# mazpie/genrl

Measured on AMD Instinct MI355X. Metric: world-model+imag update steps/sec (B32xL32x64x64x3), higher is better.
Workload: dtype f32 (storage, accumulation, every non-GEMM kernel and the fp32-MFMA GEMMs; the forward / dgrad / weight-gradient products of the imagination rollout, of the Dense+LN+SiLU chains from 192 rows up and of the encoder / decoder convolutions take fp32 operands pre-split into two fp16 planes of the scaled

## Files before the change

### genrl_amd/csrc/gemm_planes_tn.hip

```cpp
#include "common.h"
#include "genrl_hip.h"
#include <type_traits>

typedef _Float16 tn_f16x8 __attribute__((ext_vector_type(8)));
typedef _Float16 tn_f16x4 __attribute__((ext_vector_type(4)));

namespace {

struct TnArgs {
  const u16* a; long a_ld, a_plane;
  const u16* b; long b_ld, b_plane;
  const u16* fac;
  long fac_stride;
  const float* cref;
  float* out; long ldo; long split_stride;
  const float* bias_unused;
  int NI, NJ, M, stages_per_split, accumulate, tiles_i, tiles_j;
  const unsigned* rowoff; int cW, cC, ck;
};

__device__ __forceinline__ void tn_glds16(const void* g, unsigned lds_byte_addr) {
  __builtin_amdgcn_global_load_lds((const __attribute__((address_space(1))) void*)g,
                                   (__attribute__((address_space(3))) void*)(uintptr_t)lds_byte_addr, 16, 0, 0);
}
// ... 158 lines not shown
    const int s = u / (NPL * TN), p = (u / TN) % NPL, j = u % TN;
    fr[set][s][TM + j][p] = fr[set][s][TM + j][p] * fc[set][s];
  };
  auto mfma_one = [&](int set, int m) __attribute__((always_inline)) {
    constexpr int PA[3] = {1, 0, 0}, PB[3] = {0, 0, 1}, CL[3] = {0, 1, 0};
    const int s = m / (3 * TM * TN), t = (m / (TM * TN)) % 3, i = (m / TN) % TM, j = m % TN;
    acc[CL[t]][i][j] = __builtin_amdgcn_mfma_f32_32x32x16_f16(fr[set][s][TM + j][PB[t]], fr[set][s][i][PA[t]], acc[CL[t]][i][j], 0, 0, 0);
  };

  int left = nk, fleft = nk2;
  bool first = true;
  auto next_stage = [&]() __attribute__((always_inline)) {
    if (!first) {
      if (left > 0 && !(CONVB && isB)) gbase += stage_bytes;
      if (fleft > 0) fbase += BK * 2;
    }
    first = false;
    --left; --fleft;
  };
  auto issue_one = [&](int buf, int i) __attribute__((always_inline)) {
    if (i < NPD) {
      if constexpr (CONVB) {
        if (isB) { tn_glds16(gbase + (size_t)(ro[buf][i] + tapoff), piece0 + buf * STAGE + i * 1024); return; }
      }
      tn_glds16(gbase + (size_t)voff[i], piece0 + buf * STAGE + i * 1024);
    } else tn_glds4(fbase, fslot + buf * STAGE);
  };
  if constexpr (CONVB) {
    load_ro(std::integral_constant<int, 0>{});
    load_ro(std::integral_constant<int, 1>{});
    tn_wait_vm<0>();
    __builtin_amdgcn_sched_barrier(0);
  }
#pragma unroll
  for (int st = 0; st < NS; ++st) {
    next_stage();
#pragma unroll
    for (int i = 0; i < NP; ++i) issue_one(st, i);
  }
  next_stage();
  if constexpr (CONVB) {
    load_ro(std::integral_constant<int, 0>{});
    tn_wait_vm<0>();
  } else {
    tn_wait_vm<(NS - 1) * NP>();
  }
  __builtin_amdgcn_s_barrier();
  [&]<int... R>(std::integer_sequence<int, R...>) __attribute__((always_inline)) {
    (read_one(std::integral_constant<int, 0>{}, std::integral_constant<int, R>{}, std::integral_constant<int, 0>{}), ...);
  }(std::make_integer_sequence<int, TN_NR>{});
  asm volatile("s_waitcnt lgkmcnt(0)" ::: "memory");
  __builtin_amdgcn_sched_barrier(0);

  int it = 0;
  auto side_ops = [&](auto SET, auto Mc) __attribute__((always_inline)) {
    constexpr int set = decltype(SET)::value, m = decltype(Mc)::value, buf = set, buf1 = 1 - set;
    constexpr int lo = (m - TN_KB) * TN_PER;
    auto one = [&](auto Oc) __attribute__((always_inline)) {
      constexpr int o = decltype(Oc)::value;
      if constexpr (o < TN_NMEM) {
        if constexpr (tn_is_dma(o)) issue_one(buf, o / 3);
        else read_one(std::integral_constant<int, 1 - set>{}, std::integral_constant<int, (o < 3 * NP ? o - o / 3 : o - NP)>{},
                      std::integral_constant<int, buf1>{});
      }
    };
    one(std::integral_constant<int, lo>{});
    one(std::integral_constant<int, lo + 1>{});
    auto unit = [&](auto Uc) __attribute__((always_inline)) {
      constexpr int u = decltype(Uc)::value, rdy = tn_ready_of(u);
      if constexpr (rdy < TN_NM) {
        if constexpr (m == rdy) {
          constexpr int s_ = u / (NPL * TN), p_ = (u / TN) % NPL, j_ = u % TN;
          tn_wait_lgkm<tn_reads_through(m) - (tn_rlast_of(u) + 1)>(fr[1 - set][s_][TM + j_][p_], fc[1 - set][s_]);
          scale_one(1 - set, u);
        }
      } else {
        if constexpr (m == (rdy - TN_NM < TN_KB ? TN_KB : rdy - TN_NM)) scale_one(set, u);
      }
    };
    [&]<int... U>(std::integer_sequence<int, U...>) __attribute__((always_inline)) { (unit(std::integral_constant<int, U>{}), ...); }
    (std::make_integer_sequence<int, TN_NSC>{});
  };
  auto mfmas = [&](auto self, auto SET, auto Mc) __attribute__((always_inline)) -> void {
    constexpr int set = decltype(SET)::value, m = decltype(Mc)::value;
    if constexpr (m < TN_NM) {
      mfma_one(set, m);
      side_ops(SET, Mc);
      __builtin_amdgcn_sched_barrier(0);
      self(self, SET, std::integral_constant<int, m + 1>{});
    }
  };
  auto iteration = [&](auto SET) __attribute__((always_inline)) {
    constexpr int set = decltype(SET)::value;
    asm volatile("s_waitcnt lgkmcnt(0)" ::: "memory");
    __builtin_amdgcn_sched_barrier(0);
    mfma_one(set, 0);
    mfma_one(set, 1);
    __builtin_amdgcn_sched_barrier(0);
    tn_wait_vm<0>();
    __builtin_amdgcn_s_barrier();
    __builtin_amdgcn_sched_barrier(0);
    load_ro(std::integral_constant<int, 1 - set>{});
    __builtin_amdgcn_sched_barrier(0);
    mfmas(mfmas, SET, std::integral_constant<int, TN_KB>{});
    if constexpr (CONVB) { tn_wait_vm<NP>(); __builtin_amdgcn_sched_barrier(0); }
    next_stage();
    ++it;
  };
  [&]<int... U>(std::integer_sequence<int, U...>) __attribute__((always_inline)) {
    ([&](auto Uc) __attribute__((always_inline)) {
      constexpr int u = decltype(Uc)::value;
      if constexpr (tn_ready_of(u) < TN_NM) scale_one(0, u);
    }(std::integral_constant<int, U>{}), ...);
  }(std::make_integer_sequence<int, TN_NSC>{});
  while (it < nk2) {
    iteration(std::integral_constant<int, 0>{});
    iteration(std::integral_constant<int, 1>{});
  }
  tn_wait_vm<0>();

  const int l32 = lane & 31, h32 = lane >> 5;
  const float cr = g.cref[split];
  float* out = g.out + (long)split * g.split_stride;
  const bool vec = ((g.ldo & 3) == 0) && ((reinterpret_cast<uintptr_t>(out) & 15) == 0);
#pragma unroll
  for (int i = 0; i < TM; ++i) {
    const int row = i0 + (wm * TM + i) * 32 + l32;
    if (row >= g.NI) continue;
#pragma unroll
    for (int j = 0; j < TN; ++j)
#pragma unroll
      for (int gq = 0; gq < 4; ++gq) {
        const int col = j0 + (wn * TN + j) * 32 + 8 * gq + 4 * h32;
        if (col >= g.NJ) continue;
        float o[4];
#pragma unroll
        for (int v = 0; v < 4; ++v) o[v] = (acc[0][i][j][4 * gq + v] * (1.f / 2048.f) + acc[1][i][j][4 * gq + v]) * cr;
        float* c = out + (long)row * g.ldo + col;
        if (vec && col + 3 < g.NJ) {
          if (g.accumulate) {
            const float4 cv = *reinterpret_cast<const float4*>(c);
            o[0] += cv.x; o[1] += cv.y; o[2] += cv.z; o[3] += cv.w;
          }
          *reinterpret_cast<float4*>(c) = make_float4(o[0], o[1], o[2], o[3]);
        } else {
#pragma unroll
          for (int v = 0; v < 4; ++v)
            if (col + v < g.NJ) c[v] = o[v] + (g.accumulate ? c[v] : 0.f);
        }
      }
  }
}

__global__ __launch_bounds__(256) void tn_factors_kernel(const float* __restrict__ ia, const float* __restrict__ ib, int M,
                                                         int rows_per_split, long fac_stride, u16* __restrict__ fac,
                                                         float* __restrict__ cref) {
  __shared__ int red[4];
  const int r0 = blockIdx.x * rows_per_split, r1 = min(M, r0 + rows_per_split);
  auto efield = [](float v) { return (int)((__builtin_bit_cast(unsigned, v) >> 23) & 255u); };
  int emax = 0;
  for (int r = r0 + 4 * threadIdx.x; r < r1; r += 1024) {
    const float4 a = *reinterpret_cast<const float4*>(ia + r), b = *reinterpret_cast<const float4*>(ib + r);
    emax = max(max(max(efield(a.x) + efield(b.x), efield(a.y) + efield(b.y)), max(efield(a.z) + efield(b.z), efield(a.w) + efield(b.w))), emax);
  }
#pragma unroll
  for (int o = 32; o > 0; o >>= 1) emax = max(emax, __shfl_xor(emax, o, 64));
  if ((threadIdx.x & 63) == 0) red[threadIdx.x >> 6] = emax;
  __syncthreads();
  emax = max(max(red[0], red[1]), max(red[2], red[3]));
  if (threadIdx.x == 0) {
    const int e = min(max(emax - 254, -149), 127);
    cref[blockIdx.x] = ldexpf(1.0f, e);
  }
  auto f16_pow2 = [](int d) -> unsigned { return d >= -14 ? (unsigned)(d + 15) << 10 : (d >= -24 ? 1u << (d + 24) : 0u); };
  u16* f = fac + (long)blockIdx.x * fac_stride;
  for (int r = 4 * threadIdx.x; r < fac_stride; r += 1024) {
    unsigned lo = 0, hi = 0;
    if (r0 + r < r1) {
      const float4 a = *reinterpret_cast<const float4*>(ia + r0 + r), b = *reinterpret_cast<const float4*>(ib + r0 + r);
      lo = f16_pow2(efield(a.x) + efield(b.x) - emax) | (f16_pow2(efield(a.y) + efield(b.y) - emax) << 16);
      hi = f16_pow2(efield(a.z) + efield(b.z) - emax) | (f16_pow2(efield(a.w) + efield(b.w) - emax) << 16);
    }
    *reinterpret_cast<uint2*>(f + r) = make_uint2(lo, hi);
  }
}

__global__ __launch_bounds__(256) void tn_reduce_kernel(const float* __restrict__ part, long split_stride, int splits,
                                                        float* __restrict__ C, long ldc, int NI, int NJ, int accumulate) {
  const long n4 = (long)NI * (NJ / 4);
  for (long idx = (long)blockIdx.x * 256 + threadIdx.x; idx < n4; idx += (long)gridDim.x * 256) {
    const int row = (int)(idx / (NJ / 4)), c4 = (int)(idx % (NJ / 4));
    const float* p = part + (long)row * NJ + 4 * c4;
    float4 s = *reinterpret_cast<const float4*>(p);
    for (int k = 1; k < splits; ++k) {
      const float4 v = *reinterpret_cast<const float4*>(p + k * split_stride);
      s.x += v.x; s.y += v.y; s.z += v.z; s.w += v.w;
    }
    float* c = C + (long)row * ldc + 4 * c4;
    if (accumulate) { s.x += c[0]; s.y += c[1]; s.z += c[2]; s.w += c[3]; }
    c[0] = s.x; c[1] = s.y; c[2] = s.z; c[3] = s.w;
  }
}

int tn_splits(int NI, int NJ, int M) {
  const int tiles = cdiv(NI, 128) * cdiv(NJ, 128), stages = M / 64;
  int smax = stages / 8 > 0 ? stages / 8 : 1;
  if (smax > 64) smax = 64;
  int best = 1; long bc = -1;
  for (int s = 1; s <= smax; ++s) {
    const long cost = (long)cdiv((long)tiles * s, 256) * (cdiv(stages, s) + 8);
    if (bc < 0 || cost < bc) { bc = cost; best = s; }
  }
  return best;
}
struct TnPlan { int nsplit, sps; long fac_stride, fac_bytes; };
TnPlan tn_plan(int NI, int NJ, int M) {
  TnPlan p;
  const int splits = tn_splits(NI, NJ, M), stages = M / 64;
  p.sps = cdiv(stages, splits);
  p.nsplit = cdiv(stages, p.sps);
  p.fac_stride = (long)(((p.sps + 1) & ~1) * 64 + 128);
  p.fac_bytes = (p.nsplit * p.fac_stride * 2 + 255) / 256 * 256;
  return p;
}

}

extern unsigned g_planes_route;
extern int g_planes_route_splits;

extern "C" {

long genrl_gemm_h2_tn_ws_bytes(int NI, int NJ, int M) {
  if (NI <= 0 || NJ <= 0 || M <= 0) return 0;
  const TnPlan p = tn_plan(NI, NJ, M);
  long b = p.fac_bytes + 256;
  if (p.nsplit > 1) b += (long)p.nsplit * NI * ((NJ + 3) / 4 * 4) * 4;
  return b;
}

static int tn_impl(const uint16_t* a, long a_ld, long a_plane, const float* a_inv, const uint16_t* b, long b_ld, long b_plane,
                   const float* b_inv, float* C, long ldc, int NI, int NJ, int M, int accumulate, void* ws, long ws_bytes,
                   const unsigned* rowoff, int cW, int cC, int ck, void* stream) {
  GENRL_ENTER();
  if (NI <= 0 || NJ <= 0 || M <= 0 || (M & 63) || (a_ld & 63) || a_ld < NI || !a_inv || !b_inv || !ws) return GENRL_EINVAL;
  if (!rowoff && ((b_ld & 63) || b_ld < NJ)) return GENRL_EINVAL;
  if (rowoff && ((cC & 7) || (b_ld & 7) || b_ld < cC || (NJ & 7) || NJ != ck * ck * cC)) return GENRL_EINVAL;
  if (ws_bytes < genrl_gemm_h2_tn_ws_bytes(NI, NJ, M) || (reinterpret_cast<uintptr_t>(ws) & 255)) return GENRL_EINVAL;
  if ((reinterpret_cast<uintptr_t>(a_inv) | reinterpret_cast<uintptr_t>(b_inv)) & 15) return GENRL_EINVAL;
  hipStream_t s = (hipStream_t)stream;
  const TnPlan pl = tn_plan(NI, NJ, M);
  const int nsplit = pl.nsplit, sps = pl.sps;
  if (nsplit > 1 && ((NJ & 3) || (ldc & 3))) return GENRL_EINVAL;
  g_planes_route = rowoff ? GENRL_ROUTE_TN_CONV : GENRL_ROUTE_TN;
  g_planes_route_splits = nsplit;
  char* w = reinterpret_cast<char*>(ws);
  u16* fac = reinterpret_cast<u16*>(w);
  float* cref = reinterpret_cast<float*>(w + pl.fac_bytes);
  float* part = cref + 64;
  tn_factors_kernel<<<nsplit, 256, 0, s>>>(a_inv, b_inv, M, sps * 64, pl.fac_stride, fac, cref);
  GENRL_CHECK_LAUNCH();
  const int ti = cdiv(NI, 128), tj = cdiv(NJ, 128);
  const int NJp = (NJ + 3) / 4 * 4;
  TnArgs g{a, a_ld, a_plane, b, b_ld, b_plane, fac, pl.fac_stride, cref, nullptr, 0, 0, nullptr, NI, NJ, M, sps, 0, ti, tj,
           rowoff, cW, cC, ck};
  if (nsplit == 1) {
    g.out = C; g.ldo = ldc; g.split_stride = 0; g.accumulate = accumulate;
  } else {
    g.out = part; g.ldo = NJp; g.split_stride = (long)NI * NJp; g.accumulate = 0;
  }
  genrl_log_launch(rowoff ? "h2tn/conv" : "h2tn", NI, NJ, M,
                   4.0 * ((double)M * NI + (rowoff ? 4.0 * (double)M * cC : (double)M * NJ) + (double)NI * NJ));
  if (rowoff) gemm_planes_tn_kernel<true><<<ti * tj * nsplit, 256, 0, s>>>(g);
  else gemm_planes_tn_kernel<false><<<ti * tj * nsplit, 256, 0, s>>>(g);
  GENRL_CHECK_LAUNCH();
  if (nsplit > 1) {
    const long n4 = (long)NI * (NJ / 4);
    int nb = cdiv(n4, 256); if (nb > 2048) nb = 2048;
    tn_reduce_kernel<<<nb, 256, 0, s>>>(part, g.split_stride, nsplit, C, ldc, NI, NJ, accumulate);
    GENRL_CHECK_LAUNCH();
  }
  return GENRL_OK;
}

int genrl_gemm_h2_tn(const uint16_t* a, long a_ld, long a_plane, const float* a_inv, const uint16_t* b, long b_ld, long b_plane,
                     const float* b_inv, float* C, long ldc, int NI, int NJ, int M, int accumulate, void* ws, long ws_bytes,
                     void* stream) {
  g_planes_route = 0; g_planes_route_splits = 0;
  return tn_impl(a, a_ld, a_plane, a_inv, b, b_ld, b_plane, b_inv, C, ldc, NI, NJ, M, accumulate, ws, ws_bytes, nullptr, 0, 0, 0, stream);
}

int genrl_gemm_h2_tn_conv(const uint16_t* a, long a_ld, long a_plane, const float* a_inv, const uint16_t* img, long ld_img,
                          long plane_img, const float* img_inv, const unsigned* rowoff, int W, int Cc, int k, float* C, long ldc,
                          int NI, int M, int accumulate, void* ws, long ws_bytes, void* stream) {
  g_planes_route = 0; g_planes_route_splits = 0;
  if (!rowoff || k <= 0) return GENRL_EINVAL;
  return tn_impl(a, a_ld, a_plane, a_inv, img, ld_img, plane_img, img_inv, C, ldc, NI, k * k * Cc, M, accumulate, ws, ws_bytes, rowoff,
                 W, Cc, k, stream);
}

}
```

### genrl_amd/planes.py

```python
import ctypes
import os
import weakref
import torch
from ._lib import lib, check, GenrlHipError

ENABLED = os.environ.get('GENRL_PLANES', '1') != '0'
_amp_saved = None
gemm_profile = None


from .streams import raw_current_stream as _stream
from .streams import timed_start, timed_end


def r64(k):
    return (k + 63) // 64 * 64


class Planes:
    __slots__ = ('t', 'inv', 'rows', 'cols', 'ld', 'plane', 'uniform')

    def __init__(self, rows, cols, dev, zero=True):
        self.rows, self.cols, self.ld = rows, cols, r64(cols)
        self.uniform = False
# ... 71 lines not shown
        return
    arr = (_Desc * len(stale))()
    for d, ((_, transpose, c0, c1), ent) in zip(arr, stale):
        W, P = ent[3](), ent[1]
        d.src, d.ldx, d.R, d.Cn = W.data_ptr() + 4 * c0 * W.stride(1), W.stride(0), W.shape[0], c1 - c0
        d.out, d.ld_out, d.plane, d.inv, d.transpose = P.ptr(0), P.ld, P.plane, P.inv_ptr(0), int(transpose)
    check(lib().genrl_split_h2_batch(ctypes.cast(arr, ctypes.c_void_p), len(stale), stream), 'split_h2_batch')
    for _, ent in stale:
        ent[0], ent[2] = _epoch, ent[3]().data_ptr()


def _refresh_stale(stream):
    _split_entries([(key, ent) for key, ent in _wcache.items() if ent[0] != _epoch and ent[4] == stream and ent[3]() is not None], stream)


def refresh(params):
    ids = {id(q) for q in params}
    _split_entries([(key, ent) for key, ent in _wcache.items() if key[0] in ids and ent[3]() is not None], _stream())


def weight(W, transpose=False, c0=0, c1=None):
    c1 = W.shape[1] if c1 is None else c1
    if not isinstance(W, torch.nn.Parameter):
        return split(W.detach()[:, c0:c1], transpose)
    key = (id(W), transpose, c0, c1)
    ent = _wcache.get(key)
    st = _stream()
    if ent is None or ent[2] != W.data_ptr() or ent[3]() is not W:
        rows, cols = (c1 - c0, W.shape[0]) if transpose else (W.shape[0], c1 - c0)
        assert W.dim() == 2 and W.stride(1) == 1
        if ent is None:
            weakref.finalize(W, _wcache.pop, key, None)
        ent = _wcache[key] = [-1, Planes(rows, cols, W.device), W.data_ptr(), weakref.ref(W), st]
    ent[4] = st
    if ent[0] != _epoch:
        _refresh_stale(st)
    return ent[1]


def gemm(A, B, C, ldc, bias, M, N, accumulate=False, a_row0=0, A1=None, B1=None, a1_row0=0, c_off=0, b_row0=0, b1_row0=0):
    assert A.ld == B.ld and a_row0 + M <= A.rows and b_row0 + N <= B.rows, (A.ld, B.ld, A.rows, B.rows, M, N)
    e0 = timed_start(gemm_profile)
    k1 = 0
    a1 = b1 = (None, 0, 0, None)
    if A1 is not None:
        assert A1.ld == B1.ld and a1_row0 + M <= A1.rows and b1_row0 + N <= B1.rows
        k1 = A1.ld
        a1, b1 = (A1.ptr(a1_row0), A1.ld, A1.plane, A1.inv_ptr(a1_row0)), (B1.ptr(b1_row0), B1.ld, B1.plane, B1.inv_ptr(b1_row0))
    check(lib().genrl_gemm_h2(A.ptr(a_row0), A.ld, A.plane, A.inv_ptr(a_row0), B.ptr(b_row0), B.ld, B.plane, B.inv_ptr(b_row0),
                              A.ld, *a1, *b1, k1, C.data_ptr() + 4 * c_off, ldc, bias.data_ptr() if bias is not None else None,
                              M, N, int(accumulate), _stream()), 'gemm_h2')
    timed_end(gemm_profile, e0, M, N, A.cols + (A1.cols if A1 is not None else 0), 'kk/h2/pipe4')


LN_FUSED = os.environ.get('GENRL_GEMM_LN', '1') != '0'
_ln_ws = {}


def _ln_workspace(dev):
    d = torch.device(dev).index
    d = torch.cuda.current_device() if d is None else d
    ws = _ln_ws.get(d)
    if ws is None:
        if torch.cuda.is_current_stream_capturing():
            return None
        L = lib()
        ws = _ln_ws[d] = (torch.zeros(L.genrl_gemm_h2_ln_sync_words(), dtype=torch.int32, device=f'cuda:{d}'),
                          torch.zeros(L.genrl_gemm_h2_ln_part_floats(1024, 1024) + 4, device=f'cuda:{d}'))
    return ws


def ln_fused_here(dev=None):
    if not (LN_FUSED and ENABLED):
        return False
    from . import streams
    return not streams.on_side_stream() and _ln_workspace(dev if dev is not None else torch.cuda.current_device()) is not None


def gemm_ln_ok(M, N, dev=None):
    return LN_FUSED and ENABLED and lib().genrl_gemm_h2_ln_ok(M, N) == 1 and ln_fused_here(dev)


def gemm_ln(A, B, C, bias, M, N, gamma, beta, eps, out_p, out_row0, y=None, mean=None, rstd=None, act=True, a_row0=0, A1=None, B1=None,
            a1_row0=0, c_off=0, y_off=0, m_off=0):
    assert A.ld == B.ld and a_row0 + M <= A.rows and N <= B.rows and out_p.cols == N and out_row0 + M <= out_p.rows
    k1 = 0
    a1 = b1 = (None, 0, 0, None)
    if A1 is not None:
        assert A1.ld == B1.ld and a1_row0 + M <= A1.rows and N <= B1.rows
        k1 = A1.ld
        a1, b1 = (A1.ptr(a1_row0), A1.ld, A1.plane, A1.inv_ptr(a1_row0)), (B1.ptr(0), B1.ld, B1.plane, B1.inv_ptr(0))
    cptr = C.data_ptr() + 4 * c_off
    yptr = (y.data_ptr() + 4 * y_off) if y is not None else 0
    if (cptr | yptr | gamma.data_ptr() | beta.data_ptr() | (bias.data_ptr() if bias is not None else 0)) & 15:
        gemm(A, B, C, N, bias, M, N, a_row0=a_row0, A1=A1, B1=B1, a1_row0=a1_row0, c_off=c_off)
        mean_ = mean if mean is not None else torch.empty(M, device=C.device)
        rstd_ = rstd if rstd is not None else torch.empty(M, device=C.device)
        mo = m_off if mean is not None else 0
        check(lib().genrl_ln_act_fwd_h2(cptr, N, gamma.data_ptr(), beta.data_ptr(), yptr or None, N, mean_.data_ptr() + 4 * mo,
                                        rstd_.data_ptr() + 4 * (m_off if rstd is not None else 0), M, N, float(eps), int(act),
                                        out_p.ptr(out_row0), out_p.ld, out_p.plane, out_p.inv_ptr(out_row0), _stream()), 'ln_act_fwd_h2')
        return
    e0 = timed_start(gemm_profile)
    sync, part = _ln_workspace(C.device)
    check(lib().genrl_gemm_h2_ln(A.ptr(a_row0), A.ld, A.plane, A.inv_ptr(a_row0), B.ptr(0), B.ld, B.plane, B.inv_ptr(0), A.ld, *a1, *b1, k1,
                                 C.data_ptr() + 4 * c_off, N, bias.data_ptr() if bias is not None else None, M, N,
                                 gamma.data_ptr(), beta.data_ptr(), float(eps), int(act),
                                 (y.data_ptr() + 4 * y_off) if y is not None else None, N,
                                 (mean.data_ptr() + 4 * m_off) if mean is not None else None,
                                 (rstd.data_ptr() + 4 * m_off) if rstd is not None else None,
                                 out_p.ptr(out_row0), out_p.ld, out_p.plane, out_p.inv_ptr(out_row0),
                                 (part.data_ptr() + 15) // 16 * 16, sync.data_ptr(), _stream()), 'gemm_h2_ln')
    timed_end(gemm_profile, e0, M, N, A.cols + (A1.cols if A1 is not None else 0), 'kk/h2ln/pipe4')


def check_ln_failure():
    global LN_FUSED
    for d, (sync, part) in _ln_ws.items():
        if int(sync[0].item()) != 0:
            LN_FUSED = False
            sync.zero_(); part.zero_()
            raise GenrlHipError('genrl_gemm_h2_ln: the exchange of row statistics inside an XCD timed out (workgroups not dealt round-robin over the XCDs, or not co-resident); '
                                'the fused Dense -> LayerNorm form is now off (GENRL_GEMM_LN=0 turns it off from the start)')


def gemm_sample(A, B, C, ldc, bias, M, N, q, ldq, unimix, sample, lds, SP=None, a_row0=0, c_off=0, q_off=0, s_off=0, sp_row0=0):
    assert A.ld == B.ld and a_row0 + M <= A.rows and N <= B.rows and N % 32 == 0
    e0 = timed_start(gemm_profile)
    check(lib().genrl_gemm_h2_sample(A.ptr(a_row0), A.ld, A.plane, A.inv_ptr(a_row0), B.ptr(0), B.ld, B.plane, B.inv_ptr(0), A.ld,
                                     C.data_ptr() + 4 * c_off, ldc, bias.data_ptr() if bias is not None else None, M, N,
                                     q.data_ptr() + 4 * q_off, ldq, float(unimix), sample.data_ptr() + 4 * s_off, lds,
                                     SP.ptr(sp_row0) if SP is not None else None, SP.ld if SP is not None else 0,
                                     SP.plane if SP is not None else 0, SP.inv_ptr(sp_row0) if SP is not None else None, _stream()),
          'gemm_h2_sample')
    timed_end(gemm_profile, e0, M, N, A.cols, 'kk/h2/pipe4')


def gemm_tn(A, B, C, ldc, NI, NJ, M, accumulate=False, a_row0=0, b_row0=0, c_off=0):
    assert M % 64 == 0 and a_row0 + M <= A.rows and b_row0 + M <= B.rows and NI <= A.ld and NJ <= B.ld, (M, A.rows, B.rows)
    assert a_row0 % 4 == 0 and b_row0 % 4 == 0
    e0 = timed_start(gemm_profile)
    nb = lib().genrl_gemm_h2_tn_ws_bytes(NI, NJ, M)
    ws = torch.empty(nb + 256, dtype=torch.uint8, device=C.device)
    wp = (ws.data_ptr() + 255) // 256 * 256
    check(lib().genrl_gemm_h2_tn(A.ptr(a_row0), A.ld, A.plane, A.inv_ptr(a_row0), B.ptr(b_row0), B.ld, B.plane, B.inv_ptr(b_row0),
                                 C.data_ptr() + 4 * c_off, ldc, NI, NJ, M, int(accumulate), wp, nb, _stream()), 'gemm_h2_tn')
    timed_end(gemm_profile, e0, NI, NJ, M, 'rr/h2tn/pipe4')


TN_ENABLED = os.environ.get('GENRL_PLANES_WGRAD', '1') != '0'


def tn_min_rows():
    return int(os.environ.get('GENRL_TN_MIN_ROWS', '2048'))


def tn_ok(M, NI, NJ, ldc):
    return ENABLED and TN_ENABLED and M % 64 == 0 and M >= tn_min_rows() and NJ % 4 == 0 and ldc % 4 == 0
```

### include/genrl_hip.h

```cpp
#ifndef GENRL_HIP_H
#define GENRL_HIP_H
#include <stdint.h>
#ifdef __cplusplus
extern "C" {
#endif

long genrl_sgemm_ws_floats(int M, int N, int K);
int genrl_set_gemm_precision(int mode);
int genrl_sgemm_last_pipe(void);
int genrl_gemm_precision(void);
int genrl_sgemm(const float* A, long a_rs, long a_ks, const float* B, long b_rs, long b_ks, float* C, long ldc,
                const float* bias, int M, int N, int K, int accumulate, float* ws, long ws_floats, void* stream);

int genrl_sgemm_conv(const float* A, long a_rs, long a_ks, const float* B, long b_rs, long b_ks, float* C, long ldc,
                     const float* bias, int M, int N, int K, int accumulate, float* ws, long ws_floats, int which,
                     int img_h, int img_w, int img_c, int ksize, void* stream);

int genrl_split_h2(const float* x, long ldx, int R, int Cn, uint16_t* out, long ld_out, long plane, float* inv, int transpose,
                   void* stream);
int genrl_gemm_h2(const uint16_t* a0, long a0_ld, long a0_plane, const float* a0_inv, const uint16_t* b0, long b0_ld, long b0_plane,
                  const float* b0_inv, int k0, const uint16_t* a1, long a1_ld, long a1_plane, const float* a1_inv,
                  const uint16_t* b1, long b1_ld, long b1_plane, const float* b1_inv, int k1,
                  float* C, long ldc, const float* bias, int M, int N, int accumulate, void* stream);
int genrl_gemm_h2_sample(const uint16_t* a0, long a0_ld, long a0_plane, const float* a0_inv, const uint16_t* b0, long b0_ld,
// ... 1 lines not shown
                         const float* q, long ldq, float unimix, float* sample, long lds, uint16_t* sp, long sld, long splane,
                         float* sinv, void* stream);
int genrl_gemm_h2_ln_ok(int M, int N);
long genrl_gemm_h2_ln_part_floats(int M, int N);
long genrl_gemm_h2_ln_sync_words(void);
int genrl_gemm_h2_ln(const uint16_t* a0, long a0_ld, long a0_plane, const float* a0_inv, const uint16_t* b0, long b0_ld, long b0_plane,
                     const float* b0_inv, int k0, const uint16_t* a1, long a1_ld, long a1_plane, const float* a1_inv,
                     const uint16_t* b1, long b1_ld, long b1_plane, const float* b1_inv, int k1,
                     float* C, long ldc, const float* bias, int M, int N, const float* gamma, const float* beta, float eps, int act,
                     float* y, long ldy, float* mean, float* rstd, uint16_t* yp, long yld, long yplane, float* yinv,
                     float* part, unsigned* sync, void* stream);
int genrl_split_h2u(const float* x, long ldx, int R, int Cn, uint16_t* out, long ld_out, long plane, float* inv, float* ws,
                    void* stream);
int genrl_ln_act_fwd_h2u(const float* x, long ldx, const float* gamma, const float* beta, float* y, long ldy, float* mean,
                         float* rstd, int M, int N, float eps, int act, uint16_t* yp, long ldp, long plane, float* inv,
                         void* stream);
int genrl_ln_act_bwd_h2u(const float* dy, long lddy, const float* x, long ldx, const float* gamma, const float* beta,
                         const float* mean, const float* rstd, float* dx, long lddx, float* dgamma, float* dbeta, float* dcolsum,
                         float* ws, int M, int N, int act, int accumulate_params, uint16_t* dxp, long ldp, long plane, float* inv,
                         float* amax_ws, void* stream);
int genrl_gemm_h2_conv(const uint16_t* img, long ld_img, long plane_img, const float* img_inv, int Nimg, int H, int W, int Cc, int k,
                       const uint16_t* b, long b_ld, long b_plane, const float* b_inv, float* C, long ldc, const float* bias, int N,
                       int accumulate, void* stream);
int genrl_gemm_h2_subpixel(const uint16_t* img, long ld_img, long plane_img, const float* img_inv, int Nimg, int Hp, int Wp, int Cc, int T,
                           const uint16_t* b, long b_ld, long b_plane, const float* b_inv, float* out, int Ho, int Wo, int Co,
                           const float* bias, void* stream);
int genrl_pad_planes(const uint16_t* src, long splane, const float* sinv, uint16_t* dst, long dplane, float* dinv, int Nimg, int H, int W,
                     long ld, int pad, void* stream);
int genrl_planes_to_f32(const uint16_t* p, long ld, long plane, const float* inv, float* y, long ldy, long rows, int cols, void* stream);
int genrl_subpixel_weight(const float* W, long s_ci, long s_co, long s_tap, int Ci, int Co, int k, int T, float* Wsub, const float* bias,
                          float* bias4, void* stream);
int genrl_conv1_u8_fwd(const uint8_t* in, const float* Wp, const float* bias, float* y, int Nimg, int Hi, int Wi, int Co, int k, void* stream);
long genrl_conv1_u8_wgrad_ws_floats(int Co);
int genrl_conv1_u8_wgrad(const uint8_t* in, const float* dy, float* dWp, float* ws, int Nimg, int Hi, int Wi, int Co, int k, void* stream);
int genrl_convt_small_co_fwd(const float* x, const float* Wp, const float* bias, float* out, int Nimg, int Hi, int Wi, int Ci, int Co,
                             int k, int out_nchw, void* stream);
long genrl_convt_small_co_bwd_ws_floats(int Ci, int Co);
int genrl_convt_small_co_bwd(const float* x, const float* Wp, const float* dy, float* dx, float* dWp, float* ws, int Nimg, int Hi, int Wi,
                             int Ci, int Co, int k, void* stream);
long genrl_gru_seq_ws_floats(int B, int D);
int genrl_gru_seq_fwd(float* pre, const float* Wh, long ldw, const float* gamma, const float* beta, const float* h0, const float* mask,
                      float* out, float* hm, float* mean, float* rstd, float* ws, long ws_floats, int T, int B, int D, float eps,
                      void* stream);
int genrl_gru_seq_bwd(const float* dout, const float* pre, const float* Wh, long ldw, const float* gamma, const float* beta, const float* h0,
                      const float* mask, const float* out, const float* hm, const float* mean, const float* rstd, float* dpre, float* dha,
                      float* dhb, float* pa, float* pb, int S, float* dgamma, float* dbeta, int direct, float* gws, float* ws,
                      long ws_floats, int T, int B, int D, int* final_dh, int* final_parts, void* stream);
typedef struct { const uint16_t* p; long ld, plane; const float* inv; } genrl_planes_ref;
typedef struct {
  int H, N, S, K, D, A, AP, U, L;
  float unimix, min_std, max_std;
  float* stoch; float* deter; float* logit; float* action; float* raws;
  const float* eps; const float* q;
  genrl_planes_ref stoch_p, deter_p, act_p, x_p, o_p;
  float* x_pre; float* x; float* g_pre; float* o_pre; float* o;
  float* xm; float* xr; float* gm; float* gr; float* om; float* orr;
  genrl_planes_ref w_in_s, w_in_a, w_g_x, w_g_h, w_out, w_dist;
  const float* in_b; const float* in_g; const float* in_be; float in_eps;
  const float* gru_g; const float* gru_be;
  const float* out_b; const float* out_g; const float* out_be; float out_eps;
  const float* dist_b;
  genrl_planes_ref pw0s, pw0d;
  genrl_planes_ref pw[8]; const float* pb[8]; const float* pg[8]; const float* pbe[8]; float peps[8]; int pU[8];
  float* ppre[8]; float* py[8]; float* pmean[8]; float* prstd[8]; genrl_planes_ref pyp[8];
  const float* head_w; const float* head_b;
  float* ln_part; unsigned* ln_sync;
} genrl_rollout;
int genrl_imagine_seq_fwd(const genrl_rollout* r, void* stream);
typedef struct {
  int H, N, S, K, D, A, AP, U;
  float unimix, min_std, max_std;
  const float* logit; const float* deter; const float* raws; const float* eps; const float* x_pre; const float* g_pre; const float* o_pre;
  const float* xm; const float* xr; const float* gm; const float* gr; const float* om; const float* orr;
  float* ds; float* dd; const float* dl_in; const float* dact_all; float* d_raw;
  float* dlg; float* dov; float* do_pre; float* dg_pre; float* dx; float* dx_pre; float* dha; float* dhb;
  genrl_planes_ref dlg_p, dop_p, dg_p, dxp_p;
  genrl_planes_ref wt_dist, wt_out, wt_g_x, wt_g_h, wt_in_s;
  const float* waT;
  const float* out_g; const float* out_be; const float* gru_g; const float* gru_be; const float* in_g; const float* in_be;
} genrl_rollout_bwd;
int genrl_imagine_seq_bwd(const genrl_rollout_bwd* r, void* stream);
typedef struct {
  int H, N, S, K, D, A, AP, U, L;
  float unimix, min_std, max_std;
  float* stoch; float* deter; float* logit; float* action; float* raws; const float* eps; const float* q;
  float* x_pre; float* x; float* g_pre; float* o_pre; float* o;
  float* xm; float* xr; float* gm; float* gr; float* om; float* orr;
  const float* ws_in; const float* wa; const float* gru_w; const float* out_w; const float* dist_w;
  const float* in_b; const float* in_g; const float* in_be; float in_eps; const float* gru_g; const float* gru_be;
  const float* out_b; const float* out_g; const float* out_be; float out_eps; const float* dist_b;
  const float* pw[8]; const float* pb[8]; const float* pg[8]; const float* pbe[8]; float peps[8]; int pU[8];
  float* ppre[8]; float* py[8]; float* pmean[8]; float* prstd[8];
  const float* head_w; const float* head_b;
  float* ws; long ws_floats;
  float* ds; float* dd; const float* dl_in; const float* dact_all; float* d_raw;
  float* dlg; float* dov; float* do_pre; float* dg_pre; float* dx; float* dx_pre; float* dha; float* dhb; const float* waT;
} genrl_rollout_f32;
int genrl_imagine_seq_f32_fwd(const genrl_rollout_f32* r, void* stream);
int genrl_imagine_seq_f32_bwd(const genrl_rollout_f32* r, void* stream);

typedef struct {
  int T, B, S, K, D, U;
  float unimix, in_eps, out_eps;
  const float* w_in_s; long ld_in_s; const float* w_g; long ld_g; const float* w_o; long ld_o; const float* w_d;
  const float* in_g; const float* in_be; const float* gru_g; const float* gru_be; const float* out_g; const float* out_be;
  const float* dist_b; const float* mask; const float* q;
  const float* out_b; int opre_acc;
  int* idx; const float* w_in_sT; int fuse_sample;
  float* sm; float* xpre; float* xh; float* gpre; float* deter; float* opre; float* o; float* plog; float* pst;
  float* xm; float* xr; float* gm; float* gr; float* om; float* orr;
  float* ws; long ws_floats;
  const float* d_pst; float* dlg; float* dd; float* dov; float* dopre; float* dgpre; float* dxh; float* dxpre;
  float* dsa; float* dsb; float* dhd_a; float* dhd_b; float* dgamma; float* dbeta; float* gws; int direct;
} genrl_observe;
int genrl_observe_seq_fwd(const genrl_observe* r, void* stream);
int genrl_observe_seq_bwd(const genrl_observe* r, int* final_buf, void* stream);
long genrl_gemm_h2_tn_ws_bytes(int NI, int NJ, int M);
int genrl_gemm_h2_tn(const uint16_t* a, long a_ld, long a_plane, const float* a_inv, const uint16_t* b, long b_ld, long b_plane,
                     const float* b_inv, float* C, long ldc, int NI, int NJ, int M, int accumulate, void* ws, long ws_bytes,
                     void* stream);
int genrl_gemm_h2_tn_conv(const uint16_t* a, long a_ld, long a_plane, const float* a_inv, const uint16_t* img, long ld_img,
                          long plane_img, const float* img_inv, const unsigned* rowoff, int W, int Cc, int k, float* C, long ldc,
                          int NI, int M, int accumulate, void* ws, long ws_bytes, void* stream);
typedef struct {
  const float* src; long ldx; int R, Cn;
  uint16_t* out; long ld_out, plane; float* inv;
  int transpose;
} genrl_split_desc;
int genrl_split_h2_batch(const genrl_split_desc* descs, int n, void* stream);
int genrl_split_x3(const float* x, long ldx, int R, int Cn, uint16_t* out, long ld_out, long plane, int transpose,
                   void* stream);
int genrl_gemm_x3(const uint16_t* a0, long a0_ld, long a0_plane, const uint16_t* b0, long b0_ld, long b0_plane, int k0,
                  const uint16_t* a1, long a1_ld, long a1_plane, const uint16_t* b1, long b1_ld, long b1_plane, int k1,
                  float* C, long ldc, const float* bias, int M, int N, int accumulate, void* stream);
int genrl_planes_force_tile(int t);
long genrl_planes_last_route(void);
#define GENRL_ROUTE_64_NS3        0x1u
#define GENRL_ROUTE_64_NS2        0x2u
#define GENRL_ROUTE_64_SAMPLE     0x4u
#define GENRL_ROUTE_64_LN         0x8u
#define GENRL_ROUTE_128_PLAIN     0x10u
#define GENRL_ROUTE_128_HL        0x20u
#define GENRL_ROUTE_128_HLW       0x40u
#define GENRL_ROUTE_CONV_PLAIN    0x80u
#define GENRL_ROUTE_CONV_HL       0x100u
#define GENRL_ROUTE_CONV_HLW      0x200u
#define GENRL_ROUTE_CONV_TALL96   0x400u
#define GENRL_ROUTE_SUBPIXEL_HL   0x800u
#define GENRL_ROUTE_SUBPIXEL_HLW  0x1000u
#define GENRL_ROUTE_X3_64         0x2000u
#define GENRL_ROUTE_X3_128        0x4000u
#define GENRL_ROUTE_TN            0x8000u
#define GENRL_ROUTE_TN_CONV       0x10000u

int genrl_ln_act_fwd_h2(const float* x, long ldx, const float* gamma, const float* beta, float* y, long ldy, float* mean,
                        float* rstd, int M, int N, float eps, int act, uint16_t* yp, long ldp, long plane, float* inv,
                        void* stream);
typedef struct {
  const float* part; float* out0; float* out1; float* out2;
  int nchunk, N, np, accumulate;
} genrl_reduce_desc;
int genrl_ln_bwd_parts(int M, int N);
int genrl_reduce_params_batch(const genrl_reduce_desc* descs, int n, void* stream);
int genrl_ln_act_bwd_h2(const float* dy, long lddy, const float* x, long ldx, const float* gamma, const float* beta,
                        const float* mean, const float* rstd, float* dx, long lddx, float* dgamma, float* dbeta,
                        float* dcolsum, float* ws, int M, int N, int act, int accumulate_params, uint16_t* dxp, long ldp,
                        long plane, float* inv, void* stream);
int genrl_gru_gates_fwd_h2(const float* pre, const float* h, long ldh, const float* gamma, const float* beta,
                           float* hout, long ldo, float* hout2, const float* hout2_scale, float* mean, float* rstd,
                           int R, int D, float eps, uint16_t* hp, long ldp, long plane, float* inv, void* stream);
int genrl_gru_gates_bwd_h2(const float* dhout, long lddo, const float* dhout2, const float* dhout2_scale,
                           const float* pre, const float* h, long ldh, const float* gamma, const float* beta,
                           const float* mean, const float* rstd, float* dpre, float* dh, long lddh, float* dgamma,
                           float* dbeta, float* ws, int R, int D, int accumulate_params, const float* dhout2_parts,
                           int nparts, long part_stride, uint16_t* dprep, long ldp, long plane, float* inv, void* stream);
int genrl_actor_head_fwd_h2(const float* raw, const float* eps, float* action, float* mean, float* std, long R, int A,
                            float min_std, float max_std, long ld_action, uint16_t* ap, long ldp, long plane, float* inv,
                            void* stream);
int genrl_onehot_fwd_h2(const float* logits, const float* q, float* sample, float* probs, long G, int K, float unimix,
                        uint16_t* sp, int rowlen, long ldp, long plane, float* inv, void* stream);
int genrl_onehot_bwd_h2(const float* logits, const float* gsample, float* dlogits, long G, int K, float unimix,
                        int accumulate, uint16_t* dp, int rowlen, long ldp, long plane, float* inv, void* stream);

int genrl_sgemm_skinny_parts(const float* A, long a_rs, const float* B, long b_rs, long b_ks, float* P, long ldp,
                             long part_stride, int M, int N, int K, int nparts, void* stream);

int genrl_ln_act_fwd(const float* x, long ldx, const float* gamma, const float* beta, float* y, long ldy, float* mean,
                     float* rstd, int M, int N, float eps, int act, void* stream);
long genrl_ln_ws_floats(int M, int N);
int genrl_ln_act_bwd(const float* dy, long lddy, const float* x, long ldx, const float* gamma, const float* beta,
                     const float* mean, const float* rstd, float* dx, long lddx, float* dgamma, float* dbeta,
                     float* dcolsum, float* ws, int M, int N, int act, int accumulate_params, void* stream);
long genrl_colsum_ws_floats(int M, int N);
int genrl_colsum(const float* x, long ldx, float* out, float* ws, int M, int N, int accumulate, void* stream);

int genrl_gru_gates_fwd(const float* pre, const float* h, long ldh, const float* gamma, const float* beta,
                        float* hout, long ldo, float* hout2, const float* hout2_scale, float* mean, float* rstd,
                        int R, int D, float eps, void* stream);
int genrl_gru_gates_fwd_ld2(const float* pre, const float* h, long ldh, const float* gamma, const float* beta,
                            float* hout, long ldo, float* hout2, long ldo2, const float* hout2_scale, float* mean, float* rstd,
                            int R, int D, float eps, void* stream);
long genrl_gru_ws_floats(int R, int D);
int genrl_gru_gates_bwd(const float* dhout, long lddo, const float* dhout2, const float* dhout2_scale,
                        const float* pre, const float* h, long ldh, const float* gamma, const float* beta,
                        const float* mean, const float* rstd, float* dpre, float* dh, long lddh, float* dgamma,
                        float* dbeta, float* ws, int R, int D, int accumulate_params, const float* dhout2_parts,
                        int nparts, long part_stride, void* stream);
int genrl_gru_gates_bwd_ldp(const float* dhout, long lddo, const float* dhout2, const float* dhout2_scale,
                            const float* pre, const float* h, long ldh, const float* gamma, const float* beta,
                            const float* mean, const float* rstd, float* dpre, float* dh, long lddh, float* dgamma,
                            float* dbeta, float* ws, int R, int D, int accumulate_params, const float* dhout2_parts,
                            int nparts, long part_stride, long ldpart, void* stream);

int genrl_actor_head_fwd(const float* raw, const float* eps, float* action, float* mean, float* std, long R, int A,
                         float min_std, float max_std, long ld_action , void* stream);
int genrl_actor_head_linear_fwd(const float* y, long ldy, const float* W, const float* b, const float* eps, float* raw,
                                float* action, long R, int U, int A, float min_std, float max_std, long ld_action, uint16_t* ap,
                                long ldp, long plane, float* inv, void* stream);
int genrl_actor_head_linear_bwd(const float* dx, long lddx, const float* WaT, const float* daction_up, long ld_action,
                                const float* raw, const float* eps, float* draw, long R, int U, int A, float min_std, float max_std,
                                void* stream);
int genrl_actor_head_bwd(const float* daction, const float* raw, const float* eps, float* draw, long R, int A,
                         float min_std, float max_std, long ld_action , void* stream);

int genrl_copy2d(const float* src, long lds, float* dst, long ldd, long rows, int cols, const float* rowscale,
                 int accumulate, void* stream);

int genrl_onehot_fwd(const float* logits, const float* q, float* sample, float* probs, long G, int K, float unimix,
                     void* stream);
int genrl_onehot_bwd(const float* logits, const float* gsample, float* dlogits, long G, int K, float unimix,
                     int accumulate, void* stream);
int genrl_onehot_fwd_masked(const float* logits, const float* q, float* sample, float* sample2, int* idx2, const float* scale2, int S,
                            long G, int K, float unimix, void* stream);
int genrl_linear_sample32(const float* A, long a_ld, const float* W, long b_ld, const float* bias, float* C, long ldc, const float* q,
                          float* sample, float* sample2, int* idx2, const float* scale2, int M, int S, int Kred, float unimix,
                          void* stream);
int genrl_onehot_gather_ln_fwd(const int* idx, int S, int K, const float* wT, long ldw, float* xpre, long ldx, const float* gamma,
                               const float* beta, float* y, long ldy, float* mean, float* rstd, int M, int N, float eps, void* stream);
int genrl_onehot_bwd_masked(const float* logits, const float* gsample, const float* g2, const float* scale2, int S, float* dlogits,
                            long G, int K, float unimix, int accumulate, void* stream);
int genrl_cat_kl_fwd(const float* lp, const float* lq, float* kl, float* ent_p, float* ent_q, long R, int S, int K,
                     float unimix, void* stream);
int genrl_cat_kl_bwd(const float* lp, const float* lq, const float* gp, const float* gq, float* dlp, float* dlq, long R,
                     int S, int K, float unimix, void* stream);

int genrl_kl_balance_fwd(const float* kl, long R, float mix, float free_nats, float* loss, void* stream);
int genrl_kl_balance_bwd(const float* kl, const float* gloss, long R, float mix, float free_nats, float* gp, float* gq,
                         void* stream);

int genrl_twohot_fwd(const float* logits, long ld, const float* x, const float* buckets, float* out, long R, int mode,
                     void* stream);
int genrl_twohot_bwd(const float* logits, long ld, const float* x, const float* buckets, const float* gout,
                     float* dlogits, long ldd, long R, int mode, void* stream);

int genrl_lambda_return_fwd(const float* reward, const float* value, float* ret, int H, long N, float disc, float lam,
                            void* stream);
int genrl_lambda_return_bwd(const float* gret, float* dreward, float* dvalue, int H, long N, float disc, float lam,
                            int zero_tail, void* stream);

int genrl_mse_fwd(const float* mean, const uint8_t* obs, float* like, long Nimg, int E, void* stream);
int genrl_mse_bwd(const float* mean, const uint8_t* obs, const float* glike, float* dmean, long Nimg, int E,
                  void* stream);

int genrl_maxcos_fwd(const float* u, const float* v, const long* urow, float* out, long R, int E, void* stream);
int genrl_maxcos_bwd(const float* u, const float* v, const long* urow, const float* gout, float* dv, long R, int E,
                     void* stream);
int genrl_align_index(const float* ct, const float* ca, long* urow, int T, long N, int E, int nf, void* stream);

int genrl_im2col_s2(const void* in, float* cols, int Nimg, int Hi, int Wi, int C, int k, int in_mode, void* stream);
int genrl_col2im_s2(const float* cols, const float* bias, float* out, int Nimg, int Ha, int Wa, int C, int k,
                    int Ho_override, int Wo_override, int out_nchw, void* stream);
int genrl_transpose_last2(const float* in, float* out, long B, int P, int C, int accumulate, void* stream);

int genrl_gather_windows(const void* src, long row_bytes, long ring_rows, const long* start, int B, int T, void* dst,
                         void* stream);

int genrl_moments(const float* x, long n, float* out, void* stream);
int genrl_quantile_ema(const float* x, long n, float q0, float q1, float alpha, float* ema, float* out, void* stream);
int genrl_wmean_fwd(const float* x, const float* w, long n, float scale, float* out, void* stream);
int genrl_wmean_bwd(const float* g, const float* w, long n, float scale, float* dx, void* stream);
int genrl_actor_obj_fwd(const float* target, const float* weight, const float* offset_scale, int H, long N, float* loss,
                        float* out, void* stream);
int genrl_actor_obj_bwd(const float* g, const float* weight, const float* offset_scale, int H, long N, float* dtarget,
                        void* stream);
int genrl_normal_entropy_mean(const float* raw, long R, int A, float min_std, float max_std, float* out,
                              float* ws , void* stream);

int genrl_connector_prep(const float* video, const float* eps, float* clean, float* noisy, float* act_tm, int B, int T,
                         int E, int nf, float lam, float cscale, void* stream);
int genrl_cosdist_fwd(const float* x, const float* c, float* cosv, float* xnorm, float* out, long R, int E, void* stream);
int genrl_cosdist_bwd(const float* x, const float* c, const float* cosv, const float* xnorm, const float* g, float* dx,
                      long R, int E, void* stream);

long genrl_sqnorm_ws_floats(long n);
int genrl_grad_norm(const float* g, long n, float* norm_out, float* ws, float scale, int* step_inc, void* stream);
int genrl_adam_step(float* p, float* g, float* m, float* v, long n, const float* norm, float gscale, float clip,
                    float lr, float b1, float b2, float eps, float wd, int step, const int* step_dev, int zero_grad,
                    void* stream);
int genrl_scale(float* p, long n, float s, void* stream);

int genrl_relu_fwd_h2(const float* x, long ldx, float* y, long ldy, int M, int N, uint16_t* yp, long ldp, long plane, float* inv,
                      void* stream);
int genrl_relu_bwd_h2(const float* dy, long lddy, const float* y, long ldy, float* dx, long lddx, int M, int N, uint16_t* dxp, long ldp,
                      long plane, float* inv, void* stream);
int genrl_l2err_fwd(const float* t, long ldt, const float* p, long ldp, float* err, int M, int N, void* stream);
int genrl_l2err_bwd(const float* g, const float* err, const float* t, long ldt, const float* p, long ldp, float* dp, long lddp, int M,
// ... 31 lines not shown
```

Baseline: 47.18.

## Add fused 64x64-tile TN plane GEMM with in-kernel factors for small reductions

Adds a 64x64-tile TN (weight-gradient) plane GEMM kernel. It computes the per-row exponent factors and the scale reference inside the kernel, keeps them in LDS, and runs the whole K range without split-K. This removes the separate factors launch and the split-K reduction pass. A cost model chooses between it and the existing 128-tile split path. The minimum row count for routing to the TN path also drops from 2048 to 512, so more weight-gradient products go through TN. The risk is lower MFMA reuse per tile, and every tile recomputes the factors.

```diff
diff --git a/genrl_amd/csrc/gemm_planes_tn.hip b/genrl_amd/csrc/gemm_planes_tn.hip
--- a/genrl_amd/csrc/gemm_planes_tn.hip
+++ b/genrl_amd/csrc/gemm_planes_tn.hip
@@ -334,36 +334,206 @@
   }
 }
 
+struct TnExp4 { int e[4]; };
+__device__ __forceinline__ int tn_efield(float v) { return (int)((__builtin_bit_cast(unsigned, v) >> 23) & 255u); }
+__device__ __forceinline__ TnExp4 tn_exp4(const float* ia, const float* ib, int r) {
+  const float4 a = *reinterpret_cast<const float4*>(ia + r), b = *reinterpret_cast<const float4*>(ib + r);
+  return TnExp4{{tn_efield(a.x) + tn_efield(b.x), tn_efield(a.y) + tn_efield(b.y), tn_efield(a.z) + tn_efield(b.z), tn_efield(a.w) + tn_efield(b.w)}};
+}
+__device__ __forceinline__ int tn_max4(const TnExp4& x) { return max(max(x.e[0], x.e[1]), max(x.e[2], x.e[3])); }
+__device__ __forceinline__ int tn_block_max(int emax, int* red) {
+#pragma unroll
+  for (int o = 32; o > 0; o >>= 1) emax = max(emax, __shfl_xor(emax, o, 64));
+  if ((threadIdx.x & 63) == 0) red[threadIdx.x >> 6] = emax;
+  __syncthreads();
+  return max(max(red[0], red[1]), max(red[2], red[3]));
+}
+__device__ __forceinline__ float tn_cref_of(int emax) { return ldexpf(1.0f, min(max(emax - 254, -149), 127)); }
+__device__ __forceinline__ unsigned tn_f16_pow2(int d) { return d >= -14 ? (unsigned)(d + 15) << 10 : (d >= -24 ? 1u << (d + 24) : 0u); }
+__device__ __forceinline__ uint2 tn_fac4(const TnExp4& x, int emax) {
+  return make_uint2(tn_f16_pow2(x.e[0] - emax) | (tn_f16_pow2(x.e[1] - emax) << 16), tn_f16_pow2(x.e[2] - emax) | (tn_f16_pow2(x.e[3] - emax) << 16));
+}
+
 __global__ __launch_bounds__(256) void tn_factors_kernel(const float* __restrict__ ia, const float* __restrict__ ib, int M,
                                                          int rows_per_split, long fac_stride, u16* __restrict__ fac,
                                                          float* __restrict__ cref) {
   __shared__ int red[4];
   const int r0 = blockIdx.x * rows_per_split, r1 = min(M, r0 + rows_per_split);
-  auto efield = [](float v) { return (int)((__builtin_bit_cast(unsigned, v) >> 23) & 255u); };
   int emax = 0;
-  for (int r = r0 + 4 * threadIdx.x; r < r1; r += 1024) {
-    const float4 a = *reinterpret_cast<const float4*>(ia + r), b = *reinterpret_cast<const float4*>(ib + r);
-    emax = max(max(max(efield(a.x) + efield(b.x), efield(a.y) + efield(b.y)), max(efield(a.z) + efield(b.z), efield(a.w) + efield(b.w))), emax);
-  }
-#pragma unroll
-  for (int o = 32; o > 0; o >>= 1) emax = max(emax, __shfl_xor(emax, o, 64));
-  if ((threadIdx.x & 63) == 0) red[threadIdx.x >> 6] = emax;
-  __syncthreads();
-  emax = max(max(red[0], red[1]), max(red[2], red[3]));
-  if (threadIdx.x == 0) {
-    const int e = min(max(emax - 254, -149), 127);
-    cref[blockIdx.x] = ldexpf(1.0f, e);
-  }
-  auto f16_pow2 = [](int d) -> unsigned { return d >= -14 ? (unsigned)(d + 15) << 10 : (d >= -24 ? 1u << (d + 24) : 0u); };
+  for (int r = r0 + 4 * threadIdx.x; r < r1; r += 1024)
+    emax = max(tn_max4(tn_exp4(ia, ib, r)), emax);
+  emax = tn_block_max(emax, red);
+  if (threadIdx.x == 0) cref[blockIdx.x] = tn_cref_of(emax);
   u16* f = fac + (long)blockIdx.x * fac_stride;
   for (int r = 4 * threadIdx.x; r < fac_stride; r += 1024) {
-    unsigned lo = 0, hi = 0;
-    if (r0 + r < r1) {
-      const float4 a = *reinterpret_cast<const float4*>(ia + r0 + r), b = *reinterpret_cast<const float4*>(ib + r0 + r);
-      lo = f16_pow2(efield(a.x) + efield(b.x) - emax) | (f16_pow2(efield(a.y) + efield(b.y) - emax) << 16);
-      hi = f16_pow2(efield(a.z) + efield(b.z) - emax) | (f16_pow2(efield(a.w) + efield(b.w) - emax) << 16);
-    }
-    *reinterpret_cast<uint2*>(f + r) = make_uint2(lo, hi);
+    uint2 v = make_uint2(0u, 0u);
+    if (r0 + r < r1) v = tn_fac4(tn_exp4(ia, ib, r0 + r), emax);
+    *reinterpret_cast<uint2*>(f + r) = v;
+  }
+}
+
+constexpr int TN64_MAX_M = 4096;
+
+struct Tn64Args {
+  const u16* a; long a_ld, a_plane;
+  const u16* b; long b_ld, b_plane;
+  const float* a_inv; const float* b_inv;
+  float* out; long ldo;
+  int NI, NJ, M, accumulate, tiles_j;
+};
+
+struct Tn64Frag { tn_f16x4 alo[2], ahi[2], blo[2], bhi[2]; tn_f16x8 f; };
+
+template <int N> __device__ __forceinline__ void tn64_wait(Tn64Frag& x) {
+  asm volatile("s_waitcnt lgkmcnt(%9)"
+               : "+v"(x.alo[0]), "+v"(x.ahi[0]), "+v"(x.alo[1]), "+v"(x.ahi[1]), "+v"(x.blo[0]), "+v"(x.bhi[0]), "+v"(x.blo[1]),
+                 "+v"(x.bhi[1]), "+v"(x.f)
+               : "i"(N));
+}
+
+template <int NS>
+__global__ __launch_bounds__(256, NS <= 2 ? 2 : 1) void gemm_planes_tn64_kernel(Tn64Args g) {
+  constexpr int BK = 64, KS = BK / 16;
+  constexpr int PLANE_B = BK * 128;
+  constexpr int OP_B = 2 * PLANE_B;
+  constexpr int STAGE = 2 * OP_B;
+  constexpr int NPD = PLANE_B / 1024;
+  constexpr int FAC_OFF = NS * STAGE;
+  __shared__ __attribute__((aligned(1024))) unsigned char lds[NS * STAGE + TN64_MAX_M * 2];
+  __shared__ int red[4];
+
+  int L;
+  {
+    const int total = gridDim.x, x = blockIdx.x % 8, r = blockIdx.x / 8, q = total / 8, rem = total % 8;
+    L = (x < rem ? x * (q + 1) : rem * (q + 1) + (x - rem) * q) + r;
+  }
+  const int i0 = (L / g.tiles_j) * 64, j0 = (L % g.tiles_j) * 64;
+  const int nk = g.M / BK;
+  const int tid = threadIdx.x, lane = tid & 63;
+  const int wave = __builtin_amdgcn_readfirstlane(tid >> 6);
+  const int wm = wave >> 1, wn = wave & 1;
+  const unsigned lds0 = (unsigned)(uintptr_t)lds;
+
+  const bool isB = wave >= 2;
+  const int pl = wave & 1;
+  const long ld = isB ? g.b_ld : g.a_ld;
+  const char* gbase = reinterpret_cast<const char*>((isB ? g.b : g.a) + (long)pl * (isB ? g.b_plane : g.a_plane));
+  unsigned voff[NPD];
+  {
+    const int r_in = lane >> 3, pslot = lane & 7, lslot = pslot ^ (((r_in >> 1) & 1) << 2);
+    const int col = min((isB ? j0 : i0) + 8 * lslot, (int)ld - 8);
+#pragma unroll
+    for (int i = 0; i < NPD; ++i) voff[i] = (unsigned)(((long)(8 * i + r_in) * ld + col) * 2);
+  }
+  const unsigned stage_bytes = (unsigned)(BK * ld * 2);
+  const unsigned piece0 = lds0 + (isB ? OP_B : 0) + pl * PLANE_B;
+  auto issue_stage = [&](int buf) __attribute__((always_inline)) {
+#pragma unroll
+    for (int i = 0; i < NPD; ++i) tn_glds16(gbase + (size_t)voff[i], piece0 + buf * STAGE + i * 1024);
+    gbase += stage_bytes;
+  };
+#pragma unroll
+  for (int st = 0; st < NS - 1; ++st)
+    if (st < nk) issue_stage(st);
+
+  float cr;
+  {
+    TnExp4 ex[TN64_MAX_M / 1024];
+    int emax = 0;
+#pragma unroll
+    for (int c = 0; c < TN64_MAX_M / 1024; ++c) {
+      const int r = 4 * tid + 1024 * c;
+      if (r < g.M) { ex[c] = tn_exp4(g.a_inv, g.b_inv, r); emax = max(emax, tn_max4(ex[c])); }
+    }
+    emax = tn_block_max(emax, red);
+    cr = tn_cref_of(emax);
+#pragma unroll
+    for (int c = 0; c < TN64_MAX_M / 1024; ++c) {
+      const int r = 4 * tid + 1024 * c;
+      if (r < g.M) *reinterpret_cast<uint2*>(lds + FAC_OFF + 2 * r) = tn_fac4(ex[c], emax);
+    }
+    __syncthreads();
+  }
+
+  const int b4 = lane >> 4, j4 = (lane >> 2) & 3, c4 = lane & 3, kg = b4 >> 1, half = b4 & 1;
+  const unsigned rowb = (unsigned)((8 * kg + j4) * 128 + (c4 & 1) * 8), sw = ((j4 >> 1) & 1) << 2;
+  const unsigned a_ad = lds0 + rowb + (((wm * 4 + 2 * half + (c4 >> 1)) ^ sw) << 4);
+  const unsigned b_ad = lds0 + OP_B + rowb + (((wn * 4 + 2 * half + (c4 >> 1)) ^ sw) << 4);
+  unsigned f_ad = lds0 + FAC_OFF + 16 * kg;
+
+  f32x16 acc[2];
+#pragma unroll
+  for (int c = 0; c < 2; ++c)
+#pragma unroll
+    for (int r = 0; r < 16; ++r) acc[c][r] = 0.f;
+
+  auto read_step = [&](auto Sc, Tn64Frag& x, unsigned ab, unsigned bb) __attribute__((always_inline)) {
+    constexpr int s = decltype(Sc)::value, o = 16 * s * 128;
+    x.f = tn_read128<32 * s>(f_ad);
+    x.alo[0] = tn_read_tr<o>(ab); x.ahi[0] = tn_read_tr<o + 512>(ab);
+    x.alo[1] = tn_read_tr<o + PLANE_B>(ab); x.ahi[1] = tn_read_tr<o + PLANE_B + 512>(ab);
+    x.blo[0] = tn_read_tr<o>(bb); x.bhi[0] = tn_read_tr<o + 512>(bb);
+    x.blo[1] = tn_read_tr<o + PLANE_B>(bb); x.bhi[1] = tn_read_tr<o + PLANE_B + 512>(bb);
+  };
+  auto mfma_step = [&](Tn64Frag& x) __attribute__((always_inline)) {
+    const tn_f16x8 a0 = __builtin_shufflevector(x.alo[0], x.ahi[0], 0, 1, 2, 3, 4, 5, 6, 7);
+    const tn_f16x8 a1 = __builtin_shufflevector(x.alo[1], x.ahi[1], 0, 1, 2, 3, 4, 5, 6, 7);
+    const tn_f16x8 b0 = __builtin_shufflevector(x.blo[0], x.bhi[0], 0, 1, 2, 3, 4, 5, 6, 7) * x.f;
+    const tn_f16x8 b1 = __builtin_shufflevector(x.blo[1], x.bhi[1], 0, 1, 2, 3, 4, 5, 6, 7) * x.f;
+    acc[0] = __builtin_amdgcn_mfma_f32_32x32x16_f16(b0, a1, acc[0], 0, 0, 0);
+    acc[1] = __builtin_amdgcn_mfma_f32_32x32x16_f16(b0, a0, acc[1], 0, 0, 0);
+    acc[0] = __builtin_amdgcn_mfma_f32_32x32x16_f16(b1, a0, acc[0], 0, 0, 0);
+  };
+
+  int buf = 0, ibuf = NS - 1;
+  for (int t = 0; t < nk; ++t) {
+    const int newer = min(NS - 2, nk - 1 - t);
+    if (NS > 3 && newer == 2) tn_wait_vm<2 * NPD>();
+    else if (NS > 2 && newer == 1) tn_wait_vm<NPD>();
+    else tn_wait_vm<0>();
+    __builtin_amdgcn_s_barrier();
+    __builtin_amdgcn_sched_barrier(0);
+    if (t + NS - 1 < nk) issue_stage(ibuf);
+    const unsigned ab = a_ad + buf * STAGE, bb = b_ad + buf * STAGE;
+    Tn64Frag x0, x1;
+    read_step(std::integral_constant<int, 0>{}, x0, ab, bb);
+    read_step(std::integral_constant<int, 1>{}, x1, ab, bb);
+    tn64_wait<9>(x0); mfma_step(x0);
+    read_step(std::integral_constant<int, 2>{}, x0, ab, bb);
+    tn64_wait<9>(x1); mfma_step(x1);
+    read_step(std::integral_constant<int, 3>{}, x1, ab, bb);
+    tn64_wait<9>(x0); mfma_step(x0);
+    tn64_wait<0>(x1); mfma_step(x1);
+    __builtin_amdgcn_sched_barrier(0);
+    f_ad += BK * 2;
+    buf = buf + 1 == NS ? 0 : buf + 1;
+    ibuf = ibuf + 1 == NS ? 0 : ibuf + 1;
+  }
+  tn_wait_vm<0>();
+
+  const int l32 = lane & 31, h32 = lane >> 5;
+  const bool vec = ((g.ldo & 3) == 0) && ((reinterpret_cast<uintptr_t>(g.out) & 15) == 0);
+  const int row = i0 + wm * 32 + l32;
+  if (row >= g.NI) return;
+#pragma unroll
+  for (int gq = 0; gq < 4; ++gq) {
+    const int col = j0 + wn * 32 + 8 * gq + 4 * h32;
+    if (col >= g.NJ) continue;
+    float o[4];
+#pragma unroll
+    for (int v = 0; v < 4; ++v) o[v] = (acc[0][4 * gq + v] * (1.f / 2048.f) + acc[1][4 * gq + v]) * cr;
+    float* c = g.out + (long)row * g.ldo + col;
+    if (vec && col + 3 < g.NJ) {
+      if (g.accumulate) {
+        const float4 cv = *reinterpret_cast<const float4*>(c);
+        o[0] += cv.x; o[1] += cv.y; o[2] += cv.z; o[3] += cv.w;
+      }
+      *reinterpret_cast<float4*>(c) = make_float4(o[0], o[1], o[2], o[3]);
+    } else {
+#pragma unroll
+      for (int v = 0; v < 4; ++v)
+        if (col + v < g.NJ) c[v] = o[v] + (g.accumulate ? c[v] : 0.f);
+    }
   }
 }
 
@@ -406,6 +576,18 @@
   return p;
 }
 
+bool tn64_take(int NI, int NJ, int M) {
+  if (M > TN64_MAX_M) return false;
+  if (const char* e = getenv("GENRL_TN64")) return e[0] == '1';
+  const long t64 = (long)cdiv(NI, 64) * cdiv(NJ, 64), stages = M / 64;
+  if (t64 < 32) return false;
+  const long c64 = 55 + 6 * stages * (t64 > 256 ? t64 : 256) / 256;
+  const TnPlan p = tn_plan(NI, NJ, M);
+  const long t128 = (long)cdiv(NI, 128) * cdiv(NJ, 128);
+  const long c128 = 11 * cdiv(t128 * p.nsplit, 256) * (p.sps + 8) + 30 + (p.nsplit > 1 ? 50 : 0);
+  return c64 < c128;
+}
+
 }
 
 extern unsigned g_planes_route;
@@ -431,6 +613,18 @@
   if (ws_bytes < genrl_gemm_h2_tn_ws_bytes(NI, NJ, M) || (reinterpret_cast<uintptr_t>(ws) & 255)) return GENRL_EINVAL;
   if ((reinterpret_cast<uintptr_t>(a_inv) | reinterpret_cast<uintptr_t>(b_inv)) & 15) return GENRL_EINVAL;
   hipStream_t s = (hipStream_t)stream;
+  if (!rowoff && tn64_take(NI, NJ, M)) {
+    g_planes_route = GENRL_ROUTE_TN64;
+    g_planes_route_splits = 1;
+    const int tj = cdiv(NJ, 64), tiles = cdiv(NI, 64) * tj;
+    Tn64Args q{a, a_ld, a_plane, b, b_ld, b_plane, a_inv, b_inv, C, ldc, NI, NJ, M, accumulate, tj};
+    genrl_log_launch("h2tn/64", NI, NJ, M, 4.0 * ((double)M * NI + (double)M * NJ + (double)NI * NJ));
+    const char* ns = getenv("GENRL_TN64_NS");
+    if (ns ? ns[0] == '4' : tiles <= 256) gemm_planes_tn64_kernel<4><<<tiles, 256, 0, s>>>(q);
+    else gemm_planes_tn64_kernel<2><<<tiles, 256, 0, s>>>(q);
+    GENRL_CHECK_LAUNCH();
+    return GENRL_OK;
+  }
   const TnPlan pl = tn_plan(NI, NJ, M);
   const int nsplit = pl.nsplit, sps = pl.sps;
   if (nsplit > 1 && ((NJ & 3) || (ldc & 3))) return GENRL_EINVAL;
diff --git a/genrl_amd/planes.py b/genrl_amd/planes.py
--- a/genrl_amd/planes.py
+++ b/genrl_amd/planes.py
@@ -247,7 +247,7 @@
 
 
 def tn_min_rows():
-    return int(os.environ.get('GENRL_TN_MIN_ROWS', '2048'))
+    return int(os.environ.get('GENRL_TN_MIN_ROWS', '512'))
 
 
 def tn_ok(M, NI, NJ, ldc):
diff --git a/include/genrl_hip.h b/include/genrl_hip.h
--- a/include/genrl_hip.h
+++ b/include/genrl_hip.h
@@ -177,6 +177,7 @@
 #define GENRL_ROUTE_X3_128        0x4000u
 #define GENRL_ROUTE_TN            0x8000u
 #define GENRL_ROUTE_TN_CONV       0x10000u
+#define GENRL_ROUTE_TN64          0x20000u
 
 int genrl_ln_act_fwd_h2(const float* x, long ldx, const float* gamma, const float* beta, float* y, long ldy, float* mean,
                         float* rstd, int M, int N, float eps, int act, uint16_t* yp, long ldp, long plane, float* inv,
```

After: 47.24 (median of 2 runs). No clear change (+0.1%).
